# alibaba/euler

Measured on AMD Instinct MI355X. Metric: sampled edges/sec (whole node), 2-hop fanout=[25,10], 100M-node power-law graph, higher is better.
Workload: dtype f64; 1 GPU; synthetic RMAT-marginal power-law graph, 100000000 nodes / 1000001082 edges (min degree 1), f32 weights uniform [0.5,8), weighted CDF-inversion SampleNeighbor, fanout [25,10], 131072 uniform-random roots per step per GPU, TF dense layout; graph_bytes_per_gpu=94142539008, partitioning=none, streams=3, repeats=1, full=False, ranks=1

## Files before the change

### euler_amd/csrc/common.h

```cpp
#pragma once

#include <hip/hip_runtime.h>
#include <stdint.h>

#include <atomic>
#include <map>
#include <mutex>
#include <string>
#include <vector>

#include "../../include/euler_gpu.h"
#include "../../include/euler_gpu_measure.h"
#include "philox.h"

namespace euler_gpu {

void SetError(const std::string& msg);
int Fail(int code, const std::string& msg);

#define EG_HIP(expr)                                                        \
  do {                                                                      \
    hipError_t _e = (expr);                                                 \
    if (_e != hipSuccess)                                                   \
      return ::euler_gpu::Fail(EULER_GPU_EHIP,                              \
// ... 129 lines not shown
  int32_t partitions = 0;
  std::vector<std::pair<void*, int64_t>> allocations;
  std::vector<float> node_weight_sums;
  const int32_t* node_type_dev = nullptr;
  const int64_t* ufeat_ptr = nullptr;
  const int32_t* ufeat_idx = nullptr;
  const uint64_t* ufeat_val = nullptr;
  int32_t n_u64 = 0;
  bool feat_slot_aligned = false;
  const void* feat16 = nullptr;
  int32_t feat_dtype = 0;
  bool feat_slot_aligned8 = false;
  euler_gpu::EdgeStoreView edges{};
  bool has_edges = false;
  euler_gpu::NodeSamplerView edge_sampler{};
  std::vector<float> edge_weight_sums;
  std::vector<std::pair<void*, int64_t>> edge_allocs;
  std::pair<void*, int64_t> edge_sampler_alloc{nullptr, 0};
  std::vector<int64_t> bin_host_ptr;
  std::vector<int32_t> bin_host_idx;
  std::vector<uint8_t> bin_host_val;
  int32_t bin_host_slots = 0;
  mutable std::mutex bin_mu;
  mutable euler_gpu::FeatTable node_bin{};
  mutable bool node_bin_ready = false;
  mutable std::mutex ws_mu;
  mutable std::recursive_mutex launch_mu;
  mutable std::map<void*, std::pair<void*, size_t>> ws;
  mutable std::map<void*, int> ws_parity;
  mutable std::atomic<void*> last_stream{nullptr};
  mutable std::atomic<int> wb_tried{0};
  int64_t hw_bytes = 0, hw_lines = 0, hw_overflows = 0;
  int32_t hw_format = 0;
  std::vector<uint32_t> wb_overflow_rows;
  mutable std::atomic<int> blk_ready{0};
  struct FlowTableDense { void* p = nullptr; size_t rows = 0; uint32_t next_epoch = 1; };
  mutable std::map<void*, FlowTableDense> flow_tables;
  int32_t shards = 1;
  int32_t label_slot = -1;
  mutable std::mutex label_mu;
  mutable bool labels_ready = false;
  mutable int64_t n_labels = 0;
  mutable int64_t n_labelled = 0;
  mutable const uint64_t* label_nodes = nullptr;
  mutable const int64_t* label_start = nullptr;
  mutable std::vector<std::pair<void*, int64_t>> label_allocs;
  mutable std::vector<int64_t> label_off_host;
  mutable std::vector<uint8_t> label_bytes_host;
  mutable std::map<std::string, int64_t> label_lookup;
};

namespace euler_gpu {

int BuildGraphFromHost(const euler_gpu_host_csr* csr, int device,
                       int32_t partitions, int32_t shard_index, int32_t shards,
                       euler_gpu_graph** out);
int BuildGraphSynthetic(const euler_gpu_synth_params* p, int device,
                        int32_t partitions, int32_t shard_index, int32_t shards,
                        euler_gpu_graph** out);
int EnsureBlockedIndex(const euler_gpu_graph* g);
int BuildAliasTables(const std::vector<uint64_t>& ids, const std::vector<int32_t>& types,
                     const std::vector<float>& weights, int32_t n_types, NodeSamplerView* view,
                     std::vector<AliasEntry>* entries, std::vector<float>* sums,
                     const char* noun);
void DestroyEdgeStore(euler_gpu_graph* g);
int EnsureNodeBinary(const euler_gpu_graph* g);
void DestroyLabelIndex(euler_gpu_graph* g);
int ExclusiveScanI64(hipStream_t stream, const int64_t* in, int64_t* out, int64_t n);
int EnsureWbIndex(const euler_gpu_graph* g);
int SamplingView(const euler_gpu_graph* g, GraphView* out);
int LaunchSampleNeighborCounted(const euler_gpu_graph* g, hipStream_t stream, uint64_t seed,
                                uint32_t call_id, const uint64_t* roots, int64_t cap,
                                const uint32_t* n_dev, const int32_t* edge_types, int32_t k,
                                int32_t count, int64_t default_node, uint64_t* out_id,
                                float* out_w, int32_t* out_t);
int WalkEdgeTypes(hipStream_t st, const int32_t* edge_types_host, int32_t k, int32_t walk_len,
                  int32_t** et_dev);
int WalkOwnedStep(const euler_gpu_graph* g, hipStream_t st, uint64_t seed, uint32_t call_id,
                  const int32_t* et_dev, int32_t k, int32_t walk_len, int32_t step,
                  const uint64_t* ids_dev, int64_t n, uint64_t* out_dev);
int WalkPathsFromLevels(hipStream_t st, const int64_t* starts_dev, int64_t n, int32_t walk_len,
                        const uint64_t* const* level_ids_host, const int32_t* const* level_next_host,
                        int64_t default_node, int64_t* out_dev);
int FrontSlabs(hipStream_t st, const uint64_t* ids_dev, int64_t n_pos, const uint32_t* in_lens_dev,
               uint32_t in_stride, int32_t partitions, int32_t shards, uint32_t* dense_owner_dev,
               int64_t dense_limit, uint64_t* out_slabs_dev, uint32_t out_stride, uint32_t* out_lens_dev,
               bool write_headers, bool dedup, int32_t* pos_dev);
int WalkOwnedSlabs(const euler_gpu_graph* g, hipStream_t st, uint64_t seed, uint32_t call_id,
                   const int32_t* et_dev, int32_t k, int32_t walk_len, int32_t step,
                   const uint64_t* slabs_dev, const uint32_t* lens_dev, int32_t n_slabs, uint32_t stride,
                   uint64_t* out_dev);
int WalkPathsFromLevelsTail(hipStream_t st, const int64_t* starts_dev, int64_t n, int32_t walk_len,
                            const uint64_t* const* level_ids_host, const int32_t* const* level_next_host,
                            int64_t default_node, int64_t* out_dev, int32_t T, const uint32_t* lens_T_dev,
                            uint32_t stride, int32_t n_slabs, void* scratch_dev);
int N2vRowLens(hipStream_t st, const int32_t* idx_dev, int64_t m, int32_t* lens_dev);
int N2vIdxFromLens(hipStream_t st, const int32_t* lens_dev, int64_t m, int32_t* tmp_ends_dev, int32_t* idx_dev);
int N2vStoreColumn(hipStream_t st, const int64_t* src_dev, int64_t n, int64_t stride, int64_t col, int64_t* out_dev);
int N2vBoundOffsets(hipStream_t st, const int32_t* idx_dev, const int64_t* bounds_dev, int32_t w, int64_t* out_dev);
struct DatFeature {
  std::string name;
  int32_t type = 0, idx = 0;
// ... 56 lines not shown
```

### euler_amd/csrc/fanout_local.h

```cpp
#ifndef EULER_AMD_CSRC_FANOUT_LOCAL_H_
#define EULER_AMD_CSRC_FANOUT_LOCAL_H_

#include <hip/hip_runtime.h>

#include "k1_search.h"
#include "wb_index.h"
#include "wb_hw.h"
#include "wb_hw2.h"

namespace euler_gpu {

struct SmallDiv {
  uint32_t d, m;
  __host__ void Set(uint32_t div) { d = div; m = div <= 1 ? 0u : 0xFFFFFFFFu / div + 1u; }
  __device__ __forceinline__ uint32_t operator()(uint32_t n) const {
    return d <= 1 ? n : __umulhi(n, m);
  }
};

struct FanoutLocalArgs {
  GraphView g;
  uint64_t seed;
  const uint64_t* roots;
  int64_t n;
// ... 671 lines not shown
                                               uint64_t id[2], float w[2], uint32_t m[2]) {
  const double span0 = (double)__fsub_rn(sg0.lim_e, sg0.lim_b);
  const double span1 = (double)__fsub_rn(sg1.lim_e, sg1.lim_b);
  WbBucketDraw d[2];
  WbBucketPair(__dadd_rn(__dmul_rn(u0, span0), (double)sg0.lim_b), __dadd_rn(__dmul_rn(u1, span1), (double)sg1.lim_b),
               sg0.lim_e, sg1.lim_e, sg0.row_deg, sg0.row_total, d);
  bool cold0 = live0 && d[0].q3;
  bool cold1 = TWO && live1 && d[1].q3;
  const EdgeBlock* b0 = g.wb + sg0.wb_lo + d[0].j;
  const EdgeBlock* b1 = g.wb + sg0.wb_lo + (TWO ? d[1].j : d[0].j);
  const WbKeys k0 = WbLoadKeys(b0);
  WbKeys k1 = k0;
  if (TWO) k1 = WbLoadKeys(b1);
  id[0] = 0; id[1] = 0; w[0] = 0.f; w[1] = 0.f; m[0] = sg0.lo; m[1] = sg1.lo;
  const int32_t i0 = WbPickKeys(k0, d[0].f, &w[0], &m[0]);
  const int32_t i1 = TWO ? WbPickKeys(k1, d[1].f, &w[1], &m[1]) : 0;
  const bool hot0 = live0 && !cold0 && i0 >= 0;
  const bool hot1 = TWO && live1 && !cold1 && i1 >= 0;
  if (hot0) id[0] = b0->nbr[i0];
  if (hot1) id[1] = b1->nbr[i1];
  cold0 = live0 && !hot0;
  cold1 = TWO && live1 && !hot1;
  if (!TWO) { id[1] = 0; w[1] = 0.f; m[1] = sg1.lo; }
  ColdReplaySegs<TWO>(g, sg0, sg1, cold0, cold1, u0, u1, id, w, m);
}

template <bool TWO = true>
__device__ __forceinline__ void WbSamplePairG(const GraphView& g, const WbSeg sg, const int32_t t,
                                              const bool live, const double u0, const double u1,
                                              uint64_t id[2], float w[2], uint32_t m[2]) {
  WbSamplePairG2<TWO>(g, sg, sg, t, t, live, live, u0, u1, id, w, m);
}

struct WbRowT {
  const uint32_t* hd;
  const int32_t* te;
  const float* lim;
  const float* tsum;
  int64_t row;
  uint32_t row_lo, row_deg;
  bool valid;
};

__device__ __forceinline__ void LoadWbRowT(const GraphView& g, const uint64_t node, const int32_t mode,
                                           const int32_t* et, const int32_t k, WbRowT* r) {
  r->hd = nullptr; r->te = nullptr; r->lim = nullptr; r->tsum = nullptr;
  r->row_lo = 0; r->row_deg = 0; r->valid = false;
  r->row = FindRow(g, node);
  if (r->row < 0) return;
  const uint8_t* rec = g.trec + r->row * (int64_t)g.trec_stride;
  r->hd = reinterpret_cast<const uint32_t*>(rec);
  r->te = reinterpret_cast<const int32_t*>(rec + 8);
  r->lim = reinterpret_cast<const float*>(rec + 8 + 4 * g.T);
  r->tsum = reinterpret_cast<const float*>(rec + 8 + 8 * g.T);
  r->row_lo = r->hd[1];
  r->row_deg = (uint32_t)r->te[g.T - 1];
  if (mode == kTypeSub) {
    bool ok = true;
    for (int32_t i = 0; i < k; ++i) ok = ok && et[i] >= 0 && et[i] < g.T;
    r->valid = ok && SubTypeSum{r->tsum, et}((uint64_t)(k - 1)) != 0.f;
  } else {
    r->valid = r->tsum[g.T - 1] != 0.f;
  }
}

__device__ __forceinline__ bool WbTypedSeg(const GraphView& g, const WbRowT& r, const int32_t mode,
                                           const int32_t* et, const int32_t k, const double u_type,
                                           int32_t* t_out, WbSeg* s) {
  const int32_t t = mode == kTypeSub
      ? et[RandomSelectT(SubTypeSum{r.tsum, et}, 0, (uint64_t)(k - 1), u_type)]
      : (int32_t)RandomSelect(r.tsum, 0, (uint64_t)(g.T - 1), u_type);
  const int32_t b = t == 0 ? 0 : r.te[t - 1], e = r.te[t];
  s->wb_lo = r.hd[0];
  s->row_deg = r.row_deg;
  s->row_total = r.lim[g.T - 1];
  s->lim_e = r.lim[t];
  s->lim_b = t == 0 ? 0.f : r.lim[t - 1];
  s->lo = r.row_lo + (uint32_t)b;
  s->deg = e > b ? (uint32_t)(e - b) : 0u;
  s->row_lo = r.row_lo;
  *t_out = t;
  return e > b;
}

__device__ __forceinline__ void WbSampleTypedPair(const GraphView& g, const WbRowT& r, const int32_t mode,
                                                  const int32_t* et, const int32_t k, const uint64_t seed,
                                                  const uint32_t call, const uint64_t node,
                                                  const uint32_t jp, const bool live, const bool two,
                                                  uint64_t id[2], float w[2], uint32_t m[2],
                                                  int32_t tt[2], bool* sentinel) {
  const Philox4 pa = RngBlock(seed, call, kDomainNeighbor, node, 2u * jp);
  const Philox4 pb = RngBlock(seed, call, kDomainNeighbor, node, 2u * jp + 1u);
  WbSeg sg0, sg1;
  sg0.wb_lo = 0; sg0.row_deg = 0; sg0.lo = 0; sg0.deg = 0; sg0.row_total = 0.f; sg0.lim_b = 0.f; sg0.lim_e = 0.f; sg0.row_lo = 0;
  sg1 = sg0;
  tt[0] = -1; tt[1] = -1;
  bool ok0 = false, ok1 = false;
  if (live) {
    ok0 = WbTypedSeg(g, r, mode, et, k, UnitFromWords(pa.w[0], pa.w[1]), &tt[0], &sg0);
    if (two) ok1 = WbTypedSeg(g, r, mode, et, k, UnitFromWords(pb.w[0], pb.w[1]), &tt[1], &sg1);
    else sg1 = sg0;
  }
  WbSamplePairG2<true>(g, sg0, sg1, tt[0], tt[1], ok0, ok1, UnitFromWords(pa.w[2], pa.w[3]),
                       UnitFromWords(pb.w[2], pb.w[3]), id, w, m);
  *sentinel = live && (!ok0 || (two && !ok1));
  if (live && !ok0) { id[0] = 0; w[0] = 0.f; m[0] = r.row_lo; tt[0] = 0; }
  if (live && two && !ok1) { id[1] = 0; w[1] = 0.f; m[1] = r.row_lo; tt[1] = 0; }
}

struct WbRowT4 {
  uint32_t wb_lo, row_lo;
  int32_t te[4];
  float lim[4], ts[4];
  int64_t row;
  uint32_t row_deg;
  float row_total;
  bool valid;
};

template <typename V>
__device__ __forceinline__ V At4(const V a[4], const int32_t i) {
  return i == 0 ? a[0] : i == 1 ? a[1] : i == 2 ? a[2] : a[3];
}

struct RegSum4 {
  const float* ts;
  __device__ __forceinline__ float operator()(uint64_t i) const { return At4(ts, (int32_t)i); }
};

struct SubTypeSum4 {
  const float* ts;
  const int32_t* edge_types;
  __device__ __forceinline__ float operator()(uint64_t i) const {
    float s = 0.f;
    for (uint64_t x = 0; x <= i; ++x) {
      const int32_t t = edge_types[x];
      s = EG_FADD(s, EG_FSUB(At4(ts, t), t > 0 ? At4(ts, t - 1) : 0.f));
// ... 56 lines not shown
  const int32_t b = t == 0 ? 0 : At4(r.te, t - 1), e = At4(r.te, t);
  s->wb_lo = r.wb_lo;
  s->row_deg = r.row_deg;
  s->row_total = r.row_total;
  s->lim_e = At4(r.lim, t);
  s->lim_b = t == 0 ? 0.f : At4(r.lim, t - 1);
  s->lo = r.row_lo + (uint32_t)b;
  s->deg = e > b ? (uint32_t)(e - b) : 0u;
  s->row_lo = r.row_lo;
  *t_out = t;
  return e > b;
}

__device__ __forceinline__ void UniformSamplePairG2(const GraphView& g, const WbSeg sg0, const WbSeg sg1,
                                                    const int32_t t0, const int32_t t1, const bool live0,
                                                    const bool live1, const double u0, const double u1,
                                                    uint64_t id[2], float w[2], uint32_t m[2]) {
  const double r0 = __dadd_rn(__dmul_rn(u0, (double)__fsub_rn(sg0.lim_e, sg0.lim_b)), (double)sg0.lim_b);
  const double r1 = __dadd_rn(__dmul_rn(u1, (double)__fsub_rn(sg1.lim_e, sg1.lim_b)), (double)sg1.lim_b);
  const bool cold0 = live0 && !((double)sg0.lim_e > r0);
  const bool cold1 = live1 && !((double)sg1.lim_e > r1);
  id[0] = 0; id[1] = 0; w[0] = 0.f; w[1] = 0.f; m[0] = sg0.lo; m[1] = sg1.lo;
  if (live0 && !cold0) {
    m[0] = sg0.lo + ((uint32_t)r0 - (uint32_t)sg0.lim_b);
    id[0] = g.nbr[m[0]]; w[0] = 1.0f;
  }
  if (live1 && !cold1) {
    m[1] = sg1.lo + ((uint32_t)r1 - (uint32_t)sg1.lim_b);
    id[1] = g.nbr[m[1]]; w[1] = 1.0f;
  }
  ColdReplaySegs(g, sg0, sg1, cold0, cold1, u0, u1, id, w, m);
}

template <bool UNI = false>
__device__ __forceinline__ void WbSampleTypedPair4(const GraphView& g, const WbRowT4& r, const int32_t mode,
                                                   const int32_t* et, const int32_t k, const uint64_t seed,
                                                   const uint32_t call, const uint64_t node,
                                                   const uint32_t jp, const bool live, const bool two,
                                                   uint64_t id[2], float w[2], uint32_t m[2],
                                                   int32_t tt[2], bool* sentinel) {
  const Philox4 pa = RngBlock(seed, call, kDomainNeighbor, node, 2u * jp);
  const Philox4 pb = RngBlock(seed, call, kDomainNeighbor, node, 2u * jp + 1u);
  WbSeg sg0, sg1;
  sg0.wb_lo = 0; sg0.row_deg = 0; sg0.lo = 0; sg0.deg = 0; sg0.row_total = 0.f; sg0.lim_b = 0.f; sg0.lim_e = 0.f; sg0.row_lo = 0;
  sg1 = sg0;
  tt[0] = -1; tt[1] = -1;
  bool ok0 = false, ok1 = false;
  if (live) {
    ok0 = WbTypedSeg4(g, r, mode, et, k, UnitFromWords(pa.w[0], pa.w[1]), &tt[0], &sg0);
    if (two) ok1 = WbTypedSeg4(g, r, mode, et, k, UnitFromWords(pb.w[0], pb.w[1]), &tt[1], &sg1);
    else sg1 = sg0;
  }
  if (UNI) UniformSamplePairG2(g, sg0, sg1, tt[0], tt[1], ok0, ok1, UnitFromWords(pa.w[2], pa.w[3]),
                               UnitFromWords(pb.w[2], pb.w[3]), id, w, m);
  else WbSamplePairG2<true>(g, sg0, sg1, tt[0], tt[1], ok0, ok1, UnitFromWords(pa.w[2], pa.w[3]),
                            UnitFromWords(pb.w[2], pb.w[3]), id, w, m);
  *sentinel = live && (!ok0 || (two && !ok1));
  if (live && !ok0) { id[0] = 0; w[0] = 0.f; m[0] = r.row_lo; tt[0] = 0; }
  if (live && two && !ok1) { id[1] = 0; w[1] = 0.f; m[1] = r.row_lo; tt[1] = 0; }
}

struct FanoutLeanLds {
  uint32_t o_sid, o_c1, o_slotid, o_mask, o_sw, o_w1, o_st, o_slot, o_rvalid, o_t1, o_t2, bytes;
};
__host__ __device__ inline FanoutLeanLds FanoutLeanLayout(int32_t gr, int32_t c1, int32_t c2,
                                                          int32_t cap, bool typed = false) {
  FanoutLeanLds L;
  const uint32_t p = (uint32_t)gr * (uint32_t)c1;
  const uint32_t s = (uint32_t)cap * (uint32_t)c2;
  uint32_t o = 0;
  L.o_sid = o; o += s * 8;
  L.o_c1 = o; o += (p + (p & 1)) * 8;
  L.o_slotid = o; o += p * 8;
  L.o_mask = o; o += (uint32_t)gr * 8;
  L.o_sw = o; o += s * 4;
  L.o_w1 = o; o += p * 4;
  L.o_st = o; o += (uint32_t)cap * 4;
  L.o_slot = o; o += (p * 2 + 3) & ~3u;
  L.o_rvalid = o; o += ((uint32_t)gr + 3) & ~3u;
  L.o_t1 = o; L.o_t2 = o;
  if (typed) {
    o += (p + 3) & ~3u;
    L.o_t2 = o; o += (s + 3) & ~3u;
  }
  L.bytes = (o + 15) & ~15u;
  return L;
}
// ... 203 lines not shown
        WbRowT4 w4;
        if (WB == 3) { wt.hd = nullptr; wt.te = nullptr; wt.lim = nullptr; wt.tsum = nullptr; wt.row = -1; wt.row_lo = 0; wt.row_deg = 0; wt.valid = false; }
        if (kReg4) { w4.wb_lo = 0; w4.row_lo = 0; w4.row = -1; w4.row_deg = 0; w4.row_total = 0.f; w4.valid = false;
                       for (int i = 0; i < 4; ++i) { w4.te[i] = 0; w4.lim[i] = 0.f; w4.ts[i] = 0.f; } }
        if (in) {
          node = s_slotid[s0 + sl];
          if (kReg4) {
            LoadWbRowT4(g, node, a.type_mode, a.et2, a.k, &w4);
            lo = w4.row_lo; deg = w4.valid ? (int32_t)w4.row_deg : 0;
          } else if (WB == 3) {
            LoadWbRowT(g, node, a.type_mode, a.et2, a.k, &wt);
            lo = wt.row_lo; deg = wt.valid ? (int32_t)wt.row_deg : 0;
          } else if (kSeg) {
            LoadWbSeg(g, node, a.t2, &ws);
            lo = ws.lo; deg = (int32_t)ws.deg;
          } else {
            const int64_t row = LeanFindRow(g, node);
            if (row >= 0) {
              if (WB) {
                wr = g.wrec[row];
                lo = wr.lo; deg = (int32_t)wr.deg; total = wr.total;
              } else {
                const uint4 rec = *reinterpret_cast<const uint4*>(g.row_meta + row * 16);
                lo = rec.x; deg = (int32_t)rec.z; total = __uint_as_float(rec.w);
              }
            }
          }
        }
        const bool live = in && deg > 0 && !EG_FL_ABLATE(a, 2);
        uint64_t id[2]; float w[2]; uint32_t m[2];
        int32_t tt[2] = {a.t2, a.t2};
        bool sentinel = false;
        Philox4 pb;
        if (kReg4) WbSampleTypedPair4<WB == 5>(g, w4, a.type_mode, a.et2, a.k, a.seed, tile_call + 1u, node, xp, live,
                                        true, id, w, m, tt, &sentinel);
        else if (WB == 3) WbSampleTypedPair(g, wt, a.type_mode, a.et2, a.k, a.seed, tile_call + 1u, node, xp, live,
                                            true, id, w, m, tt, &sentinel);
        else pb = RngBlock(a.seed, tile_call + 1u, kDomainNeighbor, node, xp);
        if (kTyped) {}
        else if (WB == 6) UniformSamplePairG2(g, ws, ws, a.t2, a.t2, live, live, UnitFromWords(pb.w[0], pb.w[1]),
                                              UnitFromWords(pb.w[2], pb.w[3]), id, w, m);
        else if (WB == 2) WbSamplePairG(g, ws, a.t2, live, UnitFromWords(pb.w[0], pb.w[1]),
                                   UnitFromWords(pb.w[2], pb.w[3]), id, w, m);
        else if (WB == 1 && HW == 2) Hw2SamplePair(g.hw, g.prefix_w, g.nbr, wr, live, UnitFromWords(pb.w[0], pb.w[1]),
                                                   UnitFromWords(pb.w[2], pb.w[3]), id, w);
        else if (WB == 1 && HW == 1) HwSamplePair(g.hw, g.prefix_w, g.nbr, wr, live, UnitFromWords(pb.w[0], pb.w[1]),
                                                  UnitFromWords(pb.w[2], pb.w[3]), id, w);
        else if (WB) WbSamplePair(g.wb, g.prefix_w, g.nbr, wr, live, live, UnitFromWords(pb.w[0], pb.w[1]),
                                  UnitFromWords(pb.w[2], pb.w[3]), id, w, m);
        else if (UNIFORM) LeanSamplePairUniform(g, lo, deg, total, live, UnitFromWords(pb.w[0], pb.w[1]),
                                           UnitFromWords(pb.w[2], pb.w[3]), id, w, m);
        else LeanSamplePair(g, lo, deg, total, live, UnitFromWords(pb.w[0], pb.w[1]),
                            UnitFromWords(pb.w[2], pb.w[3]), id, w, m, EG_FL_ABLATE_BITS(a));
        if (in) {
          fl_u64x2 iv;
          iv.x = live ? id[0] : (uint64_t)a.default_node;
          iv.y = live ? id[1] : (uint64_t)a.default_node;
          *reinterpret_cast<fl_u64x2*>(s_sid + sl * c2 + 2u * xp) = iv;
          *reinterpret_cast<float2*>(s_sw + sl * c2 + 2u * xp) =
              make_float2(live ? w[0] : 0.f, live ? w[1] : 0.f);
          if (xp == 0) s_st[sl] = live ? a.t2 : -1;
          if (kTyped) {
            s_t2[sl * c2 + 2u * xp] = (int8_t)(live ? tt[0] : -1);
            s_t2[sl * c2 + 2u * xp + 1u] = (int8_t)(live ? tt[1] : -1);
          }
        }
      }
      WaveSync();
      if (EG_FL_DBG(a) && s0 == 0) t_s[3] = __builtin_readcyclecounter();
      if (a.row_index != nullptr) {
// ... 110 lines not shown
```

### euler_amd/csrc/graph_build.hip

```cpp
#include <hip/hip_runtime.h>
#include <sys/stat.h>
#include <hipcub/hipcub.hpp>

#include <algorithm>
#include <atomic>
#include <cstdlib>
#include <cmath>
#include <cstring>
#include <map>
#include <memory>
#include <mutex>
#include <sstream>

#include "device_fns.h"
#include "device_mem.h"
#include "wb_index.h"
#include "wb_hw.h"
#include "wb_hw2.h"

namespace euler_gpu {


namespace {
thread_local std::string g_last_error;
// ... 765 lines not shown
    if (g.T > 1) tsum[t] = m.type_prefix[t];
  }
}

constexpr int kWbOverflowKeep = 4096;

__global__ __launch_bounds__(256) void WbFillKernel(GraphView g, const uint32_t* wb_lo,
                                                    int64_t n_wb, EdgeBlock* wb,
                                                    unsigned long long* overflows) {
  uint32_t* ovf_rows = reinterpret_cast<uint32_t*>(overflows + 2);
  const int64_t stride = (int64_t)gridDim.x * blockDim.x;
  unsigned long long mine = 0;
  for (int64_t b = (int64_t)blockIdx.x * blockDim.x + threadIdx.x; b < n_wb; b += stride) {
    int64_t lo = 0, hi = g.n_rows;
    while (hi - lo > 1) {
      const int64_t mid = (lo + hi) >> 1;
      if ((int64_t)wb_lo[mid] <= b) lo = mid; else hi = mid;
    }
    const RowMeta m = LoadRowMeta(g, lo);
    const uint32_t deg = (uint32_t)m.type_end[g.T - 1];
    EdgeBlock e;
    if (WbBuildBlock(g.prefix_w, g.nbr, (uint32_t)m.row_ptr, deg, g.prefix_w[m.row_ptr + deg - 1],
                     (uint32_t)(b - (int64_t)wb_lo[lo]), &e)) {
      ++mine;
      const unsigned long long k = atomicAdd(overflows + 1, 1ull);
      if (k < (unsigned long long)kWbOverflowKeep) ovf_rows[k] = (uint32_t)lo;
    }
    wb[b] = e;
  }
  if (mine != 0) atomicAdd(overflows, mine);
}

template <int FORMAT>
__global__ __launch_bounds__(256) void HwFillKernel(GraphView g, const uint32_t* wb_lo, int64_t n_wb,
                                                    HwLine* hw, unsigned long long* overflows) {
  const int64_t stride = (int64_t)gridDim.x * blockDim.x;
  unsigned long long mine = 0;
  for (int64_t b = (int64_t)blockIdx.x * blockDim.x + threadIdx.x; b < n_wb; b += stride) {
    int64_t lo = 0, hi = g.n_rows;
    while (hi - lo > 1) {
      const int64_t mid = (lo + hi) >> 1;
      if ((int64_t)wb_lo[mid] <= b) lo = mid; else hi = mid;
    }
    const RowMeta m = LoadRowMeta(g, lo);
    const uint32_t deg = (uint32_t)m.type_end[g.T - 1];
    HwLine e;
    const uint32_t j = (uint32_t)(b - (int64_t)wb_lo[lo]);
    const float total = g.prefix_w[m.row_ptr + deg - 1];
    if (FORMAT == 2 ? Hw2BuildLine(g.prefix_w, g.nbr, (uint32_t)m.row_ptr, deg, total, j, &e)
                    : HwBuildLine(g.prefix_w, g.nbr, (uint32_t)m.row_ptr, deg, total, j, &e))
      ++mine;
    hw[b] = e;
  }
  if (mine != 0) atomicAdd(overflows, mine);
}

__global__ __launch_bounds__(256) void FatFillKernel(GraphView g, const uint8_t* trec, int32_t trec_stride,
                                                     uint8_t* fat) {
  const uint64_t stride = (uint64_t)gridDim.x * blockDim.x;
  for (uint64_t h = (uint64_t)blockIdx.x * blockDim.x + threadIdx.x; h <= g.hash_mask; h += stride) {
    const uint64_t key = g.hash_slots[2 * h];
    const int64_t row = (int64_t)g.hash_slots[2 * h + 1];
    uint4 a = make_uint4(0u, 0u, 0u, 0u), b = make_uint4(0u, 0xFFFFFFFFu, 0u, 0u), c = make_uint4(0u, 0u, 0u, 0u);
    if (row >= 0) {
      const uint8_t* rec = trec + row * (int64_t)trec_stride;
      const uint32_t* hd = reinterpret_cast<const uint32_t*>(rec);
      const int32_t* te = reinterpret_cast<const int32_t*>(rec + 8);
      const float* lim = reinterpret_cast<const float*>(rec + 8 + 4 * g.T);
      const RowMeta m = LoadRowMeta(g, row);
      const int32_t t1 = g.T - 1;
      a = make_uint4((uint32_t)key, (uint32_t)(key >> 32), hd[0], hd[1]);
      b = make_uint4((uint32_t)te[0], (uint32_t)te[t1], __float_as_uint(lim[0]), __float_as_uint(lim[t1]));
      c = make_uint4(__float_as_uint(m.type_prefix[0]), __float_as_uint(m.type_prefix[t1]),
                     (uint32_t)(uint64_t)row, (uint32_t)((uint64_t)row >> 32));
    }
    uint4* out = reinterpret_cast<uint4*>(fat + h * 64);
    out[0] = a; out[1] = b; out[2] = c; out[3] = make_uint4(0u, 0u, 0u, 0u);
  }
}

// ... 18 lines not shown
std::atomic<int64_t> g_wb_budget_ppm{-2};

void WbBudgetFromEnv() {
  if (g_wb_budget_bytes.load() != -2) return;
  int64_t bytes = -1, ppm = 500000;
  if (const char* e = getenv("EULER_GPU_WB_INDEX")) {
    if (e[0] == '0') bytes = 0;
  }
  if (const char* e = getenv("EULER_GPU_WB_INDEX_MAX_GB")) {
    const double gb = atof(e);
    if (gb >= 0 && bytes != 0) bytes = (int64_t)(gb * 1073741824.0);
  }
  if (const char* e = getenv("EULER_GPU_WB_INDEX_MAX_FRACTION")) {
    const double f = atof(e);
    if (f >= 0 && f <= 1) ppm = (int64_t)(f * 1e6);
  }
  g_wb_budget_ppm.store(ppm);
  g_wb_budget_bytes.store(bytes);
}

bool WbFits(size_t need) {
  WbBudgetFromEnv();
  size_t free_b = 0, total_b = 0;
  if (hipMemGetInfo(&free_b, &total_b) != hipSuccess) { (void)hipGetLastError(); return false; }
  const int64_t cap = g_wb_budget_bytes.load();
  if (cap >= 0 && need > (size_t)cap) return false;
  const double frac = (double)g_wb_budget_ppm.load() * 1e-6;
  if ((double)need > frac * (double)free_b) return false;
  return need + ((size_t)1 << 30) <= free_b;
}

std::atomic<int> g_hw_format{2};

void BuildHwSide(GraphBuilder* b, const uint32_t* wb_lo, int64_t n_wb) {
  static std::atomic<int> said{0};
  GraphView& v = b->g->view;
  auto decline = [&](const char* why) {
    (void)hipGetLastError();
    if (said.exchange(1) == 0)
      fprintf(stderr, "euler_gpu: header + window side index declined (%s); hop 2 of the fanout step keeps "
                      "the weight-bucket blocks\n", why);
  };
  const size_t bytes = (size_t)n_wb * sizeof(HwLine);
  if (!WbFits(bytes)) { decline("over the index budget"); return; }
  DevBuf cnt;
  AllocList side("");
  HwLine* hw = side.Alloc<HwLine>((size_t)n_wb);
  if (hw == nullptr || cnt.alloc(16) != hipSuccess || hipMemset(cnt.as(), 0, 16) != hipSuccess) {
    side.Release();
    decline("no memory");
    return;
  }
  const int format = g_hw_format.load() == 2 ? 2 : 1;
  hipLaunchKernelGGL(format == 2 ? HwFillKernel<2> : HwFillKernel<1>, dim3(GridFor(n_wb, 256)), dim3(256), 0, 0, v,
                     wb_lo, n_wb, hw, cnt.as<unsigned long long>());
  unsigned long long n_ovf = 0;
  if (hipGetLastError() != hipSuccess || hipDeviceSynchronize() != hipSuccess ||
      hipMemcpy(&n_ovf, cnt.as(), 8, hipMemcpyDeviceToHost) != hipSuccess) {
    side.Release();
    decline("build failed");
    return;
  }
  if ((double)n_ovf > 0.002 * (double)n_wb) {
    side.Release();
    decline("more than 2 lines in a thousand overflow");
    return;
  }
  for (auto& blk : side.list) b->list.push_back(blk);
  side.list.clear();
  v.hw = hw;
  b->g->hw_bytes = (int64_t)std::max<size_t>(bytes, 16);
  b->g->hw_lines = n_wb;
  b->g->hw_overflows = (int64_t)n_ovf;
  b->g->hw_format = format;
}

int BuildWbIndex(GraphBuilder* b) {
  GraphView& v = b->g->view;
  if (v.monotone != 0 && v.uniform_w != 0 && (v.T > 1 || v.map_mode != 0) && v.n_rows > 0 && v.n_edges > 0 &&
      v.n_edges < ((int64_t)1 << 31)) {
    const int32_t stride = v.T == 1 ? 16 : 8 + 12 * v.T;
    if (!WbFits((size_t)v.n_rows * stride)) return EULER_GPU_OK;
    uint8_t* trec = b->Alloc<uint8_t>((size_t)v.n_rows * stride + 16);
    if (b->rc != EULER_GPU_OK) return b->rc;
    hipLaunchKernelGGL(WbRecKernel, dim3((v.n_rows + 255) / 256), dim3(256), 0, 0, v, (const uint32_t*)nullptr,
                       trec, stride);
    EG_HIP(hipGetLastError());
    EG_HIP(hipDeviceSynchronize());
// ... 22 lines not shown
    EG_HIP(hipcub::DeviceScan::ExclusiveSum(scan_buf.as(), tmp_bytes, nbk, wb_lo, v.n_rows + 1));
    EG_HIP(hipDeviceSynchronize());
  }
  uint32_t n_wb32 = 0;
  EG_HIP(hipMemcpy(&n_wb32, wb_lo + v.n_rows, 4, hipMemcpyDeviceToHost));
  const int64_t n_wb = (int64_t)n_wb32;
  const int32_t stride = v.T == 1 ? 16 : 8 + 12 * v.T;
  if (!WbFits((size_t)n_wb * sizeof(EdgeBlock) + (size_t)v.n_rows * stride)) return EULER_GPU_OK;
  uint8_t* wbg = b->Alloc<uint8_t>((size_t)v.n_rows * stride + 16);
  static_assert(offsetof(WbRec, lo) == 4 && offsetof(WbRec, deg) == 8 && offsetof(WbRec, total) == 12,
                "WbRec is the general record at T = 1");
  const WbRec* rec = plain ? reinterpret_cast<const WbRec*>(wbg) : nullptr;
  EdgeBlock* wb = b->Alloc<EdgeBlock>((size_t)n_wb);
  if (b->rc != EULER_GPU_OK) return b->rc;
  hipLaunchKernelGGL(WbRecKernel, dim3((v.n_rows + block - 1) / block), dim3(block), 0, 0, v, wb_lo,
                     wbg, stride);
  EG_HIP(ovf_buf.alloc(16 + 4 * kWbOverflowKeep));
  unsigned long long* ovf = ovf_buf.as<unsigned long long>();
  EG_HIP(hipMemset(ovf, 0, 16 + 4 * kWbOverflowKeep));
  if (n_wb > 0)
    hipLaunchKernelGGL(WbFillKernel, dim3(GridFor(n_wb, block)), dim3(block), 0, 0, v, wb_lo, n_wb, wb, ovf);
  EG_HIP(hipGetLastError());
  EG_HIP(hipDeviceSynchronize());
  unsigned long long n_ovf = 0;
  EG_HIP(hipMemcpy(&n_ovf, ovf, 8, hipMemcpyDeviceToHost));
  {
    const size_t keep = (size_t)std::min<unsigned long long>(n_ovf, (unsigned long long)kWbOverflowKeep);
    b->g->wb_overflow_rows.resize(keep);
    if (keep > 0) EG_HIP(hipMemcpy(b->g->wb_overflow_rows.data(), ovf + 2, keep * 4, hipMemcpyDeviceToHost));
  }
  v.wrec = rec; v.wb = wb; v.n_wb = n_wb; v.wbg = wbg; v.wbg_stride = stride;
  v.trec = wbg; v.trec_stride = stride;
  v.wb_lean_ok = (double)n_ovf <= 0.002 * (double)n_wb ? 1 : 0;
  if (plain && v.has_zero_nbr == 0 && v.wb_lean_ok != 0 && n_wb > 0) BuildHwSide(b, wb_lo, n_wb);
  return BuildFatSlots(b);
}

int EnsureWbIndex(const euler_gpu_graph* cg) {
  euler_gpu_graph* g = const_cast<euler_gpu_graph*>(cg);
  if (g->wb_tried.load(std::memory_order_acquire) != 0) return EULER_GPU_OK;
  std::lock_guard<std::mutex> lk(g_blocked_mu);
  if (g->wb_tried.load(std::memory_order_acquire) != 0) return EULER_GPU_OK;
  DeviceGuard dg(g->device);
  GraphBuilder b;
  b.g.reset(g);
  const int rc = BuildWbIndex(&b);
  if (rc == EULER_GPU_OK) b.Commit();
  b.g.release();
  if (rc != EULER_GPU_OK) {
    (void)hipGetLastError();
    (void)hipDeviceSynchronize();
    (void)hipGetLastError();
    b.Release();
    GraphView& v = g->view;
    v.wb = nullptr; v.wbg = nullptr; v.wrec = nullptr; v.n_wb = 0; v.wb_lean_ok = 0;
    v.trec = nullptr; v.trec_stride = 0; v.fat = nullptr;
    v.hw = nullptr; g->hw_bytes = 0; g->hw_lines = 0; g->hw_overflows = 0; g->hw_format = 0;
  }
  g->wb_tried.store(1, std::memory_order_release);
  return EULER_GPU_OK;
}

std::atomic<int> g_blk_fail_next{0};

int EnsureBlockedIndex(const euler_gpu_graph* cg) {
  euler_gpu_graph* g = const_cast<euler_gpu_graph*>(cg);
  if (g->blk_ready.load(std::memory_order_acquire) != 0) return EULER_GPU_OK;
  std::lock_guard<std::mutex> lk(g_blocked_mu);
  if (g->blk_ready.load(std::memory_order_acquire) != 0) return EULER_GPU_OK;
  DeviceGuard dg(g->device);
  GraphBuilder b;
  b.g.reset(g);
  int rc;
  if (g_blk_fail_next.load() > 0) {
    g_blk_fail_next.fetch_sub(1);
    (void)b.Alloc<uint8_t>(4096);
    rc = Fail(EULER_GPU_ENOMEM, "EdgeBlocks: allocation failure injected (tuning key 56)");
  } else {
    rc = BuildBlockedIndex(&b);
  }
  if (rc == EULER_GPU_OK) b.Commit();
  b.g.release();
  if (rc != EULER_GPU_OK) {
    (void)hipGetLastError();
    (void)hipDeviceSynchronize();
    (void)hipGetLastError();
    b.Release();
    GraphView& v = g->view;
    v.blk = nullptr; v.skip1 = nullptr; v.bpiv = nullptr; v.n_blk = 0;
  }
  g->blk_ready.store(rc == EULER_GPU_OK ? 1 : 2, std::memory_order_release);
  return EULER_GPU_OK;
// ... 367 lines not shown
```

### euler_amd/csrc/sample_kernels.hip

```cpp
#include <hip/hip_runtime.h>
#include <hipcub/hipcub.hpp>

#include <cmath>
#include <vector>

#include "device_mem.h"
#include "k1_args.h"
#include "k1_search.h"
#include "fanout_local.h"
#include "fanout_plain.h"

extern thread_local int g_feature_vec4;
namespace euler_gpu { extern thread_local int g_walk_collapse, g_walk_grid, g_walk_tail, g_walk_lean; extern std::atomic<int> g_walk_path_ch, g_n2v_list_big, g_n2v_list_big_parent, g_n2v_list_merged, g_n2v_walk_tickets; }
namespace euler_gpu { extern std::atomic<int> g_sharded_self_exchange, g_sharded_walk_enqueued, g_sharded_walk_tail, g_sharded_walk_split; }
namespace euler_gpu { extern std::atomic<int> g_flow_fused; extern std::atomic<int> g_flow_rowpos; }
namespace euler_gpu { extern std::atomic<int> g_blk_fail_next; }
namespace euler_gpu { extern std::atomic<int> g_hw_format; }
namespace euler_gpu { extern thread_local int g_label_hash_bits; }
namespace euler_gpu { extern thread_local int g_root_host_batch, g_adj_scan, g_adj_long_row, g_sum_scalar; }

namespace euler_gpu {

struct DedupArgs {
  GraphView g;
// ... 1312 lines not shown
            int64_t pwaves = g_fl_grid_cap > 0 ? g_fl_grid_cap : 0;
            if (pwaves > 0 && pblocks > (pwaves + pwpb - 1) / pwpb) pblocks = (pwaves + pwpb - 1) / pwpb;
            void (*pk)(const FanoutPlainArgs) = nullptr;
#define EG_FP(W) (hw2 == 2 ? SampleFanoutPlainKernel<W, 2> : hw2 == 1 ? SampleFanoutPlainKernel<W, 1> : SampleFanoutPlainKernel<W, 0>)
            pk = g_fp_wps >= 8 ? EG_FP(8) : g_fp_wps == 7 ? EG_FP(7) : g_fp_wps == 6 ? EG_FP(6)
                 : g_fp_wps == 5 ? EG_FP(5) : EG_FP(4);
#undef EG_FP
            t_fl_took_lean = 1;
            t_fl_last_kernel = "SampleFanoutPlainKernel";
            hipLaunchKernelGGL(pk, dim3((unsigned)pblocks), dim3(pblock), (size_t)pl.bytes * pwpb, stream, pa);
            EG_HIP(hipGetLastError());
            if (uniq_off != nullptr) { uniq_off[0] = -1; uniq_off[1] = -1; }
            return EULER_GPU_OK;
          }
        }
        if (!big && (size_t)ll.bytes * (block / 64) <= 64 * 1024) {
          f.cap = lcap; f.wave_lds = (int32_t)ll.bytes;
          f.div_h1.Set((uint32_t)(c1 + 1) / 2); f.div_h2.Set((uint32_t)c2 / 2);
          const size_t llds = (size_t)ll.bytes * wpb;
#ifdef EULER_GPU_MEASURE
          f.dbg = (unsigned long long*)g_fl_debug;
          f.ablate = g_fl_ablate;
#endif
          f.row_index = t_fl_row_index;
          t_fl_took_lean = 1;
          void (*lk)(const FanoutLocalArgs) = nullptr;
          const bool use_wb = v.uniform_w == 0 && f.g.wrec != nullptr && f.g.wb != nullptr && v.wb_lean_ok != 0;
#define EG_LW(W, ...) (f.wide ? SampleFanoutLeanKernel<true, W, __VA_ARGS__> : SampleFanoutLeanKernel<false, W, __VA_ARGS__>)
#define EG_LEAN_5(...) EG_LW(5, __VA_ARGS__)
#define EG_LEAN_65(...) (g_fl_wps == 6 ? EG_LW(6, __VA_ARGS__) : EG_LW(5, __VA_ARGS__))
#define EG_LEAN_85(...) (g_fl_wps == 8 ? EG_LW(8, __VA_ARGS__) : EG_LW(5, __VA_ARGS__))
#define EG_LEAN_856(...) (g_fl_wps == 8 ? EG_LW(8, __VA_ARGS__) : g_fl_wps == 5 ? EG_LW(5, __VA_ARGS__) : EG_LW(6, __VA_ARGS__))
          const bool side = use_wb && plain && g_fp_hw != 0 && f.g.hw != nullptr;
          if (lean_gu) lk = EG_LEAN_5(false, 6, 0);
          else if (lean_tu) lk = EG_LEAN_5(false, 5, 0);
          else if (lean_t && v.T <= 4 && g_fl_typed_regs != 0) lk = EG_LEAN_5(false, 4, 0);
          else if (lean_t) lk = EG_LEAN_5(false, 3, 0);
          else if (lean_g) lk = EG_LEAN_65(false, 2, 0);
          else if (v.uniform_w != 0) lk = EG_LEAN_85(true, 0, 0);
          else if (side && g->hw_format == 2) lk = EG_LEAN_856(false, 1, 2);
          else if (side) lk = EG_LEAN_856(false, 1, 1);
          else if (use_wb) lk = EG_LEAN_856(false, 1, 0);
          else lk = EG_LEAN_856(false, 0, 0);
#undef EG_LEAN_856
#undef EG_LEAN_85
#undef EG_LEAN_65
#undef EG_LEAN_5
#undef EG_LW
          t_fl_last_kernel = "SampleFanoutLeanKernel";
          hipLaunchKernelGGL(lk, dim3((unsigned)blocks), dim3(block), llds, stream, f);
          EG_HIP(hipGetLastError());
          if (uniq_off != nullptr) { uniq_off[0] = -1; uniq_off[1] = -1; }
          return EULER_GPU_OK;
        }
      }
      if (!lean_only && !big) {
      void (*kern)(const FanoutLocalArgs) = nullptr;
#define EG_FL(W, P) (g_fl_wps != 8 ? SampleFanoutLocalKernel<W, P, 5> : SampleFanoutLocalKernel<W, P, 8>)
      kern = f.wide ? (plain ? EG_FL(true, true) : EG_FL(true, false))
                    : (plain ? EG_FL(false, true) : EG_FL(false, false));
#undef EG_FL
      t_fl_last_kernel = "SampleFanoutLocalKernel";
      hipLaunchKernelGGL(kern, dim3((unsigned)blocks), dim3(block), lds, stream, f);
      EG_HIP(hipGetLastError());
      if (uniq_off != nullptr) { uniq_off[0] = -1; uniq_off[1] = -1; }
      return EULER_GPU_OK;
      }
    }
// ... 773 lines not shown
```

### euler_amd/csrc/wb_hw2.h

```cpp
#ifndef EULER_AMD_CSRC_WB_HW2_H_
#define EULER_AMD_CSRC_WB_HW2_H_

#include "wb_hw.h"

namespace euler_gpu {

constexpr uint32_t kHw2In = 4093;
constexpr uint32_t kHw2Max = 4094;
constexpr uint32_t kHw2Pad = 4095;

EG_HD uint32_t Hw2Code(float v) {
  const float m = EG_FMUL(v, (float)kHw2Max);
  const uint32_t q = !(m >= 0.f) ? 0u : (m < (float)kHw2Max ? (uint32_t)m : kHw2In);
  return v >= 1.f ? kHw2Max : q;
}

EG_HD float Hw2Pos(float x, float scale, uint32_t j) { return EG_FSUB(EG_FMUL(x, scale), (float)j); }

EG_HD bool Hw2BuildLine(const float* prefix_w, const uint64_t* nbr, uint32_t lo, uint32_t deg,
                        float total, uint32_t j, HwLine* out) {
  const uint32_t nbk = WbBuckets(deg);
  const ArraySum nw{prefix_w + lo};
  const float scale = WbScale(nbk, total);
  const uint32_t s = WbBlockStart(nw, deg, nbk, scale, j);
// ... 36 lines not shown
  uint32_t i = 0;
  i += (h.c0 & 4095u) <= t ? 1u : 0u;
  i += ((h.c0 >> 12) & 4095u) <= t ? 1u : 0u;
  i += ((h.c0 >> 24) | ((h.c1 & 15u) << 8)) <= t ? 1u : 0u;
  i += ((h.c1 >> 4) & 4095u) <= t ? 1u : 0u;
  i += ((h.c1 >> 16) & 4095u) <= t ? 1u : 0u;
  i += ((h.c1 >> 28) | ((h.c2 & 255u) << 4)) <= t ? 1u : 0u;
  i += ((h.c2 >> 8) & 4095u) <= t ? 1u : 0u;
  i += (h.c2 >> 20) <= t ? 1u : 0u;
  return i;
}

EG_HD int32_t Hw2Draw(const HwLine* ln, float f, uint32_t t, uint64_t* id, float* w) {
  const uint32_t i = Hw2Guess(Hw2LoadHead(ln), t);
  const int32_t d = HwCheck(HwLoadWin(ln, i), f, id, w);
  if (d == 0) return 1;
  if (d > 0 || i == 0u) return -1;
  return HwCheck(HwLoadWin(ln, i - 1u), f, id, w) == 0 ? 2 : -2;
}

EG_HD bool Hw2SampleHot(const HwLine* hw, const WbRec& rec, double u, uint64_t* id, float* w,
                        int32_t* windows) {
  const double r = EG_DMUL(u, (double)rec.total);
  *windows = 0;
  if (!((double)rec.total > r)) return false;
  const float f = WbFloorToFloat(r);
  const uint32_t nbk = WbBuckets(rec.deg);
  const float scale = WbScale(nbk, rec.total);
  const uint32_t j = nbk <= 1u ? 0u : WbBucketOf(f, nbk, scale);
  *windows = Hw2Draw(hw + rec.wb_lo + j, f, Hw2Code(Hw2Pos(f, scale, j)), id, w);
  return *windows > 0;
}

}

#endif
```

Baseline: 196.8 billion sampled edges/s.

## Use HW2 line side-table for typed weighted neighbor sampling in lean kernel

Adds a lazily built HW2 line side-table for typed (non-plain) graphs, built from the blocked wbg rows via a strided wb_lo lookup. The typed lean fanout kernel now uses these packed lines when present: it guesses a window from 12-bit codes and falls back to cold replay. This replaces the wider bucket search. It costs extra device memory and a one-time build, and it only helps if the workload takes the typed lean path.

Result: slower. 194.6 billion sampled edges/s (-1.2%).

```diff
diff --git a/euler_amd/csrc/common.h b/euler_amd/csrc/common.h
--- a/euler_amd/csrc/common.h
+++ b/euler_amd/csrc/common.h
@@ -185,6 +185,7 @@
   mutable std::atomic<int> wb_tried{0};
   int64_t hw_bytes = 0, hw_lines = 0, hw_overflows = 0;
   int32_t hw_format = 0;
+  mutable std::atomic<int> hw_tried{0};
   std::vector<uint32_t> wb_overflow_rows;
   mutable std::atomic<int> blk_ready{0};
   struct FlowTableDense { void* p = nullptr; size_t rows = 0; uint32_t next_epoch = 1; };
@@ -221,6 +222,7 @@
 void DestroyLabelIndex(euler_gpu_graph* g);
 int ExclusiveScanI64(hipStream_t stream, const int64_t* in, int64_t* out, int64_t n);
 int EnsureWbIndex(const euler_gpu_graph* g);
+int EnsureHwSide(const euler_gpu_graph* g);
 int SamplingView(const euler_gpu_graph* g, GraphView* out);
 int LaunchSampleNeighborCounted(const euler_gpu_graph* g, hipStream_t stream, uint64_t seed,
                                 uint32_t call_id, const uint64_t* roots, int64_t cap,
diff --git a/euler_amd/csrc/fanout_local.h b/euler_amd/csrc/fanout_local.h
--- a/euler_amd/csrc/fanout_local.h
+++ b/euler_amd/csrc/fanout_local.h
@@ -727,6 +727,36 @@
   WbSamplePairG2<TWO>(g, sg, sg, t, t, live, live, u0, u1, id, w, m);
 }
 
+__device__ __forceinline__ void Hw2SamplePairG2(const HwLine* hw, const GraphView& g, const WbSeg sg0,
+                                                const WbSeg sg1, const bool live0, const bool live1,
+                                                const double u0, const double u1, uint64_t id[2], float w[2]) {
+  const uint32_t nbk = WbBuckets(sg0.row_deg);
+  const float scale = WbScale(nbk, sg0.row_total);
+  const Hw2SegDraw d0 = Hw2SegPrepare(u0, sg0.lim_b, sg0.lim_e, nbk, scale);
+  const Hw2SegDraw d1 = Hw2SegPrepare(u1, sg1.lim_b, sg1.lim_e, nbk, scale);
+  const bool t0 = live0 && d0.below, t1 = live1 && d1.below;
+  const HwLine* l0 = hw + sg0.wb_lo + d0.j;
+  const HwLine* l1 = hw + sg0.wb_lo + d1.j;
+  const Hw2Head h0 = Hw2LoadHead(l0), h1 = Hw2LoadHead(l1);
+  const uint32_t i0 = Hw2Guess(h0, d0.t), i1 = Hw2Guess(h1, d1.t);
+  const HwWin x0 = HwLoadWin(l0, i0), x1 = HwLoadWin(l1, i1);
+  id[0] = 0; id[1] = 0; w[0] = 0.f; w[1] = 0.f;
+  const int32_t c0 = HwCheck(x0, d0.f, &id[0], &w[0]), c1 = HwCheck(x1, d1.f, &id[1], &w[1]);
+  bool hot0 = t0 && c0 == 0, hot1 = t1 && c1 == 0;
+  const bool ask0 = t0 && c0 < 0 && i0 != 0u, ask1 = t1 && c1 < 0 && i1 != 0u;
+  if (__ballot(ask0 || ask1) != 0ull) {
+    HwWin y0{0u, 0u, 0u, 0u}, y1{0u, 0u, 0u, 0u};
+    if (ask0) y0 = HwLoadWin(l0, i0 - 1u);
+    if (ask1) y1 = HwLoadWin(l1, i1 - 1u);
+    const int32_t e0 = HwCheck(y0, d0.f, &id[0], &w[0]), e1 = HwCheck(y1, d1.f, &id[1], &w[1]);
+    hot0 = hot0 || (ask0 && e0 == 0);
+    hot1 = hot1 || (ask1 && e1 == 0);
+  }
+  if (!hot0) { id[0] = 0; w[0] = 0.f; }
+  if (!hot1) { id[1] = 0; w[1] = 0.f; }
+  ColdReplaySegs<true>(g, sg0, sg1, live0 && !hot0, live1 && !hot1, u0, u1, id, w, nullptr);
+}
+
 struct WbRowT {
   const uint32_t* hd;
   const int32_t* te;
@@ -778,6 +808,7 @@
   return e > b;
 }
 
+template <int HW = 0>
 __device__ __forceinline__ void WbSampleTypedPair(const GraphView& g, const WbRowT& r, const int32_t mode,
                                                   const int32_t* et, const int32_t k, const uint64_t seed,
                                                   const uint32_t call, const uint64_t node,
@@ -796,8 +827,14 @@
     if (two) ok1 = WbTypedSeg(g, r, mode, et, k, UnitFromWords(pb.w[0], pb.w[1]), &tt[1], &sg1);
     else sg1 = sg0;
   }
-  WbSamplePairG2<true>(g, sg0, sg1, tt[0], tt[1], ok0, ok1, UnitFromWords(pa.w[2], pa.w[3]),
-                       UnitFromWords(pb.w[2], pb.w[3]), id, w, m);
+  if (HW == 2) {
+    m[0] = r.row_lo; m[1] = r.row_lo;
+    Hw2SamplePairG2(g.hw, g, sg0, sg1, ok0, ok1, UnitFromWords(pa.w[2], pa.w[3]), UnitFromWords(pb.w[2], pb.w[3]),
+                    id, w);
+  } else {
+    WbSamplePairG2<true>(g, sg0, sg1, tt[0], tt[1], ok0, ok1, UnitFromWords(pa.w[2], pa.w[3]),
+                         UnitFromWords(pb.w[2], pb.w[3]), id, w, m);
+  }
   *sentinel = live && (!ok0 || (two && !ok1));
   if (live && !ok0) { id[0] = 0; w[0] = 0.f; m[0] = r.row_lo; tt[0] = 0; }
   if (live && two && !ok1) { id[1] = 0; w[1] = 0.f; m[1] = r.row_lo; tt[1] = 0; }
@@ -920,7 +957,7 @@
   ColdReplaySegs(g, sg0, sg1, cold0, cold1, u0, u1, id, w, m);
 }
 
-template <bool UNI = false>
+template <bool UNI = false, int HW = 0>
 __device__ __forceinline__ void WbSampleTypedPair4(const GraphView& g, const WbRowT4& r, const int32_t mode,
                                                    const int32_t* et, const int32_t k, const uint64_t seed,
                                                    const uint32_t call, const uint64_t node,
@@ -941,6 +978,11 @@
   }
   if (UNI) UniformSamplePairG2(g, sg0, sg1, tt[0], tt[1], ok0, ok1, UnitFromWords(pa.w[2], pa.w[3]),
                                UnitFromWords(pb.w[2], pb.w[3]), id, w, m);
+  else if (HW == 2) {
+    m[0] = r.row_lo; m[1] = r.row_lo;
+    Hw2SamplePairG2(g.hw, g, sg0, sg1, ok0, ok1, UnitFromWords(pa.w[2], pa.w[3]), UnitFromWords(pb.w[2], pb.w[3]),
+                    id, w);
+  }
   else WbSamplePairG2<true>(g, sg0, sg1, tt[0], tt[1], ok0, ok1, UnitFromWords(pa.w[2], pa.w[3]),
                             UnitFromWords(pb.w[2], pb.w[3]), id, w, m);
   *sentinel = live && (!ok0 || (two && !ok1));
@@ -1210,10 +1252,10 @@
         int32_t tt[2] = {a.t2, a.t2};
         bool sentinel = false;
         Philox4 pb;
-        if (kReg4) WbSampleTypedPair4<WB == 5>(g, w4, a.type_mode, a.et2, a.k, a.seed, tile_call + 1u, node, xp, live,
-                                        true, id, w, m, tt, &sentinel);
-        else if (WB == 3) WbSampleTypedPair(g, wt, a.type_mode, a.et2, a.k, a.seed, tile_call + 1u, node, xp, live,
+        if (kReg4) WbSampleTypedPair4<WB == 5, HW>(g, w4, a.type_mode, a.et2, a.k, a.seed, tile_call + 1u, node, xp, live,
                                             true, id, w, m, tt, &sentinel);
+        else if (WB == 3) WbSampleTypedPair<HW>(g, wt, a.type_mode, a.et2, a.k, a.seed, tile_call + 1u, node, xp, live,
+                                                true, id, w, m, tt, &sentinel);
         else pb = RngBlock(a.seed, tile_call + 1u, kDomainNeighbor, node, xp);
         if (kTyped) {}
         else if (WB == 6) UniformSamplePairG2(g, ws, ws, a.t2, a.t2, live, live, UnitFromWords(pb.w[0], pb.w[1]),
diff --git a/euler_amd/csrc/graph_build.hip b/euler_amd/csrc/graph_build.hip
--- a/euler_amd/csrc/graph_build.hip
+++ b/euler_amd/csrc/graph_build.hip
@@ -821,20 +821,20 @@
 }
 
 template <int FORMAT>
-__global__ __launch_bounds__(256) void HwFillKernel(GraphView g, const uint32_t* wb_lo, int64_t n_wb,
-                                                    HwLine* hw, unsigned long long* overflows) {
+__global__ __launch_bounds__(256) void HwFillKernel(GraphView g, const uint32_t* wb_lo, int64_t lo_stride,
+                                                    int64_t n_wb, HwLine* hw, unsigned long long* overflows) {
   const int64_t stride = (int64_t)gridDim.x * blockDim.x;
   unsigned long long mine = 0;
   for (int64_t b = (int64_t)blockIdx.x * blockDim.x + threadIdx.x; b < n_wb; b += stride) {
     int64_t lo = 0, hi = g.n_rows;
     while (hi - lo > 1) {
       const int64_t mid = (lo + hi) >> 1;
-      if ((int64_t)wb_lo[mid] <= b) lo = mid; else hi = mid;
+      if ((int64_t)wb_lo[mid * lo_stride] <= b) lo = mid; else hi = mid;
     }
     const RowMeta m = LoadRowMeta(g, lo);
     const uint32_t deg = (uint32_t)m.type_end[g.T - 1];
     HwLine e;
-    const uint32_t j = (uint32_t)(b - (int64_t)wb_lo[lo]);
+    const uint32_t j = (uint32_t)(b - (int64_t)wb_lo[lo * lo_stride]);
     const float total = g.prefix_w[m.row_ptr + deg - 1];
     if (FORMAT == 2 ? Hw2BuildLine(g.prefix_w, g.nbr, (uint32_t)m.row_ptr, deg, total, j, &e)
                     : HwBuildLine(g.prefix_w, g.nbr, (uint32_t)m.row_ptr, deg, total, j, &e))
@@ -919,7 +919,7 @@
 
 std::atomic<int> g_hw_format{2};
 
-void BuildHwSide(GraphBuilder* b, const uint32_t* wb_lo, int64_t n_wb) {
+void BuildHwSide(GraphBuilder* b, const uint32_t* wb_lo, int64_t lo_stride, int64_t n_wb, int format) {
   static std::atomic<int> said{0};
   GraphView& v = b->g->view;
   auto decline = [&](const char* why) {
@@ -938,9 +938,8 @@
     decline("no memory");
     return;
   }
-  const int format = g_hw_format.load() == 2 ? 2 : 1;
   hipLaunchKernelGGL(format == 2 ? HwFillKernel<2> : HwFillKernel<1>, dim3(GridFor(n_wb, 256)), dim3(256), 0, 0, v,
-                     wb_lo, n_wb, hw, cnt.as<unsigned long long>());
+                     wb_lo, lo_stride, n_wb, hw, cnt.as<unsigned long long>());
   unsigned long long n_ovf = 0;
   if (hipGetLastError() != hipSuccess || hipDeviceSynchronize() != hipSuccess ||
       hipMemcpy(&n_ovf, cnt.as(), 8, hipMemcpyDeviceToHost) != hipSuccess) {
@@ -1029,7 +1028,8 @@
   v.wrec = rec; v.wb = wb; v.n_wb = n_wb; v.wbg = wbg; v.wbg_stride = stride;
   v.trec = wbg; v.trec_stride = stride;
   v.wb_lean_ok = (double)n_ovf <= 0.002 * (double)n_wb ? 1 : 0;
-  if (plain && v.has_zero_nbr == 0 && v.wb_lean_ok != 0 && n_wb > 0) BuildHwSide(b, wb_lo, n_wb);
+  if (plain && v.has_zero_nbr == 0 && v.wb_lean_ok != 0 && n_wb > 0)
+    BuildHwSide(b, wb_lo, 1, n_wb, g_hw_format.load() == 2 ? 2 : 1);
   return BuildFatSlots(b);
 }
 
@@ -1054,7 +1054,35 @@
     v.trec = nullptr; v.trec_stride = 0; v.fat = nullptr;
     v.hw = nullptr; g->hw_bytes = 0; g->hw_lines = 0; g->hw_overflows = 0; g->hw_format = 0;
   }
+  {
+    const GraphView& v = g->view;
+    const bool plain = v.T == 1 && v.total_in_meta != 0 && v.map_mode == 0;
+    const bool later = !plain && v.wbg != nullptr && v.wb != nullptr && v.wb_lean_ok != 0 && v.has_zero_nbr == 0 &&
+                       v.uniform_w == 0 && v.n_wb > 0;
+    if (!later) g->hw_tried.store(1, std::memory_order_release);
+  }
   g->wb_tried.store(1, std::memory_order_release);
+  return EULER_GPU_OK;
+}
+
+int EnsureHwSide(const euler_gpu_graph* cg) {
+  euler_gpu_graph* g = const_cast<euler_gpu_graph*>(cg);
+  if (g->hw_tried.load(std::memory_order_acquire) != 0) return EULER_GPU_OK;
+  const int rc = EnsureWbIndex(cg);
+  if (rc != EULER_GPU_OK) return rc;
+  std::lock_guard<std::mutex> lk(g_blocked_mu);
+  if (g->hw_tried.load(std::memory_order_acquire) != 0) return EULER_GPU_OK;
+  const GraphView& v = g->view;
+  if (g_hw_format.load() == 2 && v.wbg != nullptr && v.wb != nullptr && v.wb_lean_ok != 0 && v.has_zero_nbr == 0 &&
+      v.uniform_w == 0 && v.n_wb > 0 && v.wbg_stride % 4 == 0) {
+    DeviceGuard dg(g->device);
+    GraphBuilder b;
+    b.g.reset(g);
+    BuildHwSide(&b, reinterpret_cast<const uint32_t*>(v.wbg), v.wbg_stride / 4, v.n_wb, 2);
+    b.Commit();
+    b.g.release();
+  }
+  g->hw_tried.store(1, std::memory_order_release);
   return EULER_GPU_OK;
 }
 
diff --git a/euler_amd/csrc/sample_kernels.hip b/euler_amd/csrc/sample_kernels.hip
--- a/euler_amd/csrc/sample_kernels.hip
+++ b/euler_amd/csrc/sample_kernels.hip
@@ -1368,8 +1368,17 @@
 #define EG_LEAN_85(...) (g_fl_wps == 8 ? EG_LW(8, __VA_ARGS__) : EG_LW(5, __VA_ARGS__))
 #define EG_LEAN_856(...) (g_fl_wps == 8 ? EG_LW(8, __VA_ARGS__) : g_fl_wps == 5 ? EG_LW(5, __VA_ARGS__) : EG_LW(6, __VA_ARGS__))
           const bool side = use_wb && plain && g_fp_hw != 0 && f.g.hw != nullptr;
+          bool side_g = false;
+          if (lean_t && !lean_tu && g_fp_hw != 0) {
+            const int rc1 = EnsureHwSide(g);
+            if (rc1 != EULER_GPU_OK) return rc1;
+            f.g.hw = g->view.hw;
+            side_g = f.g.hw != nullptr && g->hw_format == 2;
+          }
           if (lean_gu) lk = EG_LEAN_5(false, 6, 0);
           else if (lean_tu) lk = EG_LEAN_5(false, 5, 0);
+          else if (lean_t && v.T <= 4 && g_fl_typed_regs != 0 && side_g) lk = EG_LW(4, false, 4, 2);
+          else if (lean_t && side_g) lk = EG_LW(4, false, 3, 2);
           else if (lean_t && v.T <= 4 && g_fl_typed_regs != 0) lk = EG_LEAN_5(false, 4, 0);
           else if (lean_t) lk = EG_LEAN_5(false, 3, 0);
           else if (lean_g) lk = EG_LEAN_65(false, 2, 0);
diff --git a/euler_amd/csrc/wb_hw2.h b/euler_amd/csrc/wb_hw2.h
--- a/euler_amd/csrc/wb_hw2.h
+++ b/euler_amd/csrc/wb_hw2.h
@@ -92,6 +92,32 @@
   return *windows > 0;
 }
 
+struct Hw2SegDraw {
+  bool below;
+  float f;
+  uint32_t j, t;
+};
+
+EG_HD Hw2SegDraw Hw2SegPrepare(double u, float lim_b, float lim_e, uint32_t nbk, float scale) {
+  Hw2SegDraw d;
+  const double r = ScaleDraw(u, lim_b, lim_e);
+  d.below = (double)lim_e > r;
+  d.f = WbFloorToFloat(r);
+  d.j = nbk <= 1u ? 0u : WbBucketOf(d.f, nbk, scale);
+  d.t = Hw2Code(Hw2Pos(d.f, scale, d.j));
+  return d;
+}
+
+EG_HD bool Hw2SampleHotSeg(const HwLine* hw, uint32_t wb_lo, uint32_t row_deg, float row_total,
+                           float lim_b, float lim_e, double u, uint64_t* id, float* w, int32_t* windows) {
+  const uint32_t nbk = WbBuckets(row_deg);
+  const Hw2SegDraw d = Hw2SegPrepare(u, lim_b, lim_e, nbk, WbScale(nbk, row_total));
+  *windows = 0;
+  if (!d.below) return false;
+  *windows = Hw2Draw(hw + wb_lo + d.j, d.f, d.t, id, w);
+  return *windows > 0;
+}
+
 }
 
 #endif
```
